# googlegenomics/spark-examples

Hardware: NVIDIA H100
Metric: genotype-cells/sec (N x V) into Gram (higher is better)
Workload: dtype int8

## Files before the change

include/vpca.h:

```cpp
#ifndef VPCA_H_
#define VPCA_H_

#include <stddef.h>
#include <stdint.h>

#ifdef __cplusplus
extern "C" {
#endif

#define VPCA_VERSION_MAJOR 0
#define VPCA_VERSION_MINOR 2

typedef enum vpca_status {
    VPCA_OK = 0,
    VPCA_ERR_BAD_ARG = -1,
    VPCA_ERR_INDEX_OUT_OF_RANGE = -2,
    VPCA_ERR_CUDA = -3,
    VPCA_ERR_NCCL = -4,
    VPCA_ERR_OVERFLOW = -5,
    VPCA_ERR_STATE = -6,
    VPCA_ERR_NOMEM = -7,
    VPCA_ERR_UNSUPPORTED = -8
} vpca_status;

// ... 152 lines not shown
    int32_t eig_method;
    int32_t eig_iterations;
} vpca_stats;
int vpca_get_stats(vpca_ctx* ctx, vpca_stats* out);
int vpca_debug_gram_profile(vpca_ctx* ctx, int64_t* out, int32_t max_ctas);
int vpca_debug_lanczos_profile(vpca_ctx* ctx, int64_t* out, int32_t max_steps);

#define VPCA_JOIN 0
#define VPCA_MERGE 1
int vpca_hash_keys(vpca_ctx* ctx, const uint8_t* payload, const int64_t* key_offsets, int64_t nkeys, uint64_t* out);
int vpca_join_rows(vpca_ctx* ctx, int32_t mode, int32_t variant_set_count, int64_t n_left, const uint8_t* key_payload,
                   const int64_t* key_offsets, const int64_t* offsets, const int32_t* sample_idx, int64_t nrows,
                   int64_t* out_rows, int64_t* out_nnz);
int vpca_join_fetch(vpca_ctx* ctx, int64_t* out_offsets, int32_t* out_idx);
int vpca_join_size(vpca_ctx* ctx, int64_t* out_rows, int64_t* out_nnz);
int vpca_accumulate_joined(vpca_ctx* ctx, int64_t partition_id);

int vpca_debug_rebalance(const int32_t* tiles, int32_t num_tiles, int32_t workers, int32_t kb_window, int32_t col_limit,
                         double* cum, int32_t* out, int32_t max_pieces);
int vpca_debug_tiles(int32_t n_samples, int32_t cta_group, int32_t exact, int32_t* out, int32_t max_tiles);
int vpca_debug_band_tiles(int32_t n_samples, int32_t cta_group, int32_t row0, int32_t rows, int32_t* out, int32_t max_tiles);
int vpca_debug_max_clusters(int32_t device, int32_t cluster_size);
int vpca_debug_plan(const int32_t* tiles, int32_t num_tiles, int32_t workers, int32_t kb_window, int32_t* out, int32_t max_pieces);

#ifdef __cplusplus
}
#endif
#endif
```

spark_examples_b200/csrc/gram_sm90.cu:

```cuda
#include <cuda.h>
#include <cuda_runtime.h>

#include <cstring>

#include <algorithm>
#include <map>
#include <mutex>
#include <tuple>
#include <type_traits>
#include <cstdio>
#include <cstdlib>
#include <string>
#include <vector>

#include "ptx_sm90.cuh"
#include "vpca_internal.h"

namespace vpca {

namespace {

constexpr int kThreads = 384;
constexpr int kKBytes = 128;
constexpr int kBoxRows = 128;
// ... 29 lines not shown
struct GramArgs {
    int32_t* S;
    int32_t* peer[kMaxPeers];
    int num_peers;
    int peer_mode;
    int own_end[kMaxPeers];
    const TileDesc* tiles;
    int* err;
    int n;
    int num_tiles;
    int num_full;
    int total_weight;
    int kb_total;
    int kb_window;
    int num_workers;
    int resident;
    int kc_per_kb;
    int kb_per_panel;
    int sync_lead;
    int active_workers;
    int* win_done;
    long long* prof;
    const double* cum;
    int col_limit;
    int acc_stride;
    int row_limit;
    int red64;
};

struct Seg {
    int tile, kb0, kb1, col, slot, first, flush, use, win, last_in_win;
    int rowA0, rowA1, rowB, n_eff, flags;
};

struct SegPlan {
    int n;
    int tile[kMaxSegs], lo[kMaxSegs], hi[kMaxSegs], col[kMaxSegs];
    int cols;
    int overflow;
};

__host__ __device__ inline void plan_segments(const TileDesc* tiles, int num_tiles, int first_tile, long long u_begin,
                                              long long u_end, int len, SegPlan& p) {
    p.n = 0;
    p.cols = 0;
    p.overflow = 0;
// ... 67 lines not shown
            int h = 0;
            if (feasible_end(tiles, num_tiles, mid, need[j + 1], len, col_limit, h) >= need[j + 1]) hi = mid;
            else lo = mid + 1;
        }
        need[j] = hi;
    }
    long long ub = 0;
    int hint = 0;
    for (int i = 0; i < workers; ++i) {
        long long ue = (i + 1 == workers) ? uw : (long long)((double)uw * cand[i + 1]);
        if (ue < ub) ue = ub;
        if (i + 1 < workers && ue < need[i + 1]) ue = need[i + 1];
        const long long fe = feasible_end(tiles, num_tiles, ub, ue, len, col_limit, hint);
        if (fe < ue) {
            if (i + 1 == workers || fe < need[i + 1]) return false;
            ue = fe;
        }
        if (i + 1 < workers) cand[i + 1] = ((double)ue + 0.5) / (double)uw;
        ub = ue;
    }
    return true;
}

struct Sched {
    SegPlan plan;
    long long u_begin, u_end, u;
    int kbw, nwin, kb_total, resident, win, seg_i, nflush, acc_stride;
    int worker, workers, num_tiles, wave, full_waves, tail_first;
    const TileDesc* tiles;

    __device__ void init(const GramArgs& a, int w) {
        kbw = a.kb_window;
        kb_total = a.kb_total;
        resident = a.resident;
        acc_stride = a.acc_stride;
        worker = w;
        workers = a.num_workers;
        num_tiles = a.num_tiles;
        tiles = a.tiles;
        nwin = (kb_total + kbw - 1) / kbw;
        win = 0;
        seg_i = 0;
        nflush = 0;
        wave = 0;
        if (resident) {
            const long long uw = (long long)a.total_weight * kbw;
            u_begin = (long long)((double)uw * a.cum[worker]);
            u_end = (worker + 1 == a.num_workers) ? uw : (long long)((double)uw * a.cum[worker + 1]);
            plan_segments(tiles, num_tiles, 0, u_begin, u_end, kbw, plan);
            if (plan.overflow || plan.cols > a.col_limit) {
                if (a.err != nullptr && threadIdx.x == 0) {
                    a.err[0] = 9;
                    a.err[1] = (int)blockIdx.x;
                    a.err[2] = plan.cols;
                    a.err[3] = plan.n;
                    __threadfence_system();
                }
                __trap();
            }
        } else {
            full_waves = a.num_full / workers;
            tail_first = full_waves * workers;
            const long long tail_units =
                tail_first < num_tiles ? (long long)(a.total_weight - tiles[tail_first].wstart) * kb_total : 0;
            u_begin = tail_units * worker / workers;
            u_end = tail_units * (worker + 1) / workers;
            plan.n = 0;
        }
        u = u_begin;
    }
    __device__ void fill(Seg& s, int t) const {
        const int4 lo = __ldg(reinterpret_cast<const int4*>(tiles + t));
        const int4 hi = __ldg(reinterpret_cast<const int4*>(tiles + t) + 1);
        s.tile = t;
        s.rowA0 = lo.x;
        s.rowA1 = lo.y;
        s.rowB = lo.z;
        s.n_eff = lo.w;
        s.flags = hi.y;
    }
    __device__ bool next(Seg& s) {
        if (!resident) {
            s.win = 0;
            s.last_in_win = 0;
            s.first = 1;
            s.flush = 1;
            s.slot = nflush & 1;
            s.col = s.slot * acc_stride;
            s.use = nflush >> 1;
            if (wave < full_waves) {
                fill(s, wave * workers + worker);
                s.kb0 = 0;
                s.kb1 = kb_total;
                ++wave;
                ++nflush;
                return true;
            }
            while (true) {
                if (seg_i < plan.n) {
                    fill(s, plan.tile[seg_i]);
                    s.kb0 = plan.lo[seg_i];
                    s.kb1 = plan.hi[seg_i];
                    ++seg_i;
                    ++nflush;
                    return true;
                }
                if (u >= u_end) return false;
                plan_segments(tiles, num_tiles, tail_first, u, u_end, kb_total, plan);
                seg_i = 0;
                if (plan.n == 0) return false;
                const int lt = plan.tile[plan.n - 1];
                const long long base = (long long)(tiles[lt].wstart - tiles[tail_first].wstart) * kb_total;
                const long long endu = base + (long long)plan.hi[plan.n - 1] * (tiles[lt].n_eff >> 4);
                u = plan.overflow ? endu : u_end;
            }
        }
        if (plan.n == 0) return false;
        if (seg_i == plan.n) {
            ++win;
            seg_i = 0;
        }
        if (win >= nwin) return false;
        const int i = seg_i++;
        fill(s, plan.tile[i]);
        const int base = win * kbw;
        const int cnt = min(kbw, kb_total - base);
        s.kb0 = base + min(plan.lo[i], cnt);
        s.kb1 = base + min(plan.hi[i], cnt);
        s.win = win;
        s.last_in_win = (seg_i == plan.n);
        s.col = plan.col[i];
        s.slot = i;
        s.first = (win == 0);
        s.flush = (win == nwin - 1);
        s.use = 0;
        return true;
    }
};

__device__ __forceinline__ void mbar_wait(uint32_t bar, uint32_t parity, int* err, int code) {
    if (ptx::mbar_try_wait(bar, parity)) return;
    const long long t0 = clock64();
    while (!ptx::mbar_try_wait(bar, parity)) {
        if (clock64() - t0 > kWatchdogCycles) {
            if (err != nullptr) {
                err[0] = code;
                err[1] = (int)blockIdx.x;
                err[2] = (int)bar;
                err[3] = (int)parity;
                __threadfence_system();
            }
// ... 345 lines not shown
        double acc = 0.0;
        cand[0] = 0.0;
        for (int i = 0; i < workers; ++i) {
            acc += sh[i] / sum;
            cand[i + 1] = (i + 1 == workers) ? 1.0 : acc;
        }
    }
    __syncthreads();
    if (active) {
        const long long uw = (long long)total_weight * kbw;
        const long long ub = (long long)((double)uw * cand[w]);
        const long long ue = (w + 1 == workers) ? uw : (long long)((double)uw * cand[w + 1]);
        int hint = 0;
        if (feasible_end(tiles, num_tiles, ub, ue, kbw, col_limit, hint) < ue) atomicExch(&need_repair, 1);
    }
    __syncthreads();
    if (need_repair && w == 0 && !repair_split(tiles, num_tiles, workers, (long long)total_weight * kbw, kbw, col_limit, cand, need)) reject = 1;
    __syncthreads();
    if (reject) return;
    if (w <= workers) cum[w] = cand[w];
    if (w == 0) *gen += 1;
}

__global__ void symmetrize_kernel(int32_t* __restrict__ S, int n) {
    __shared__ int32_t tile[32][33];
    const int bx = blockIdx.x, by = blockIdx.y;
    if (bx < by) return;
    const int tx = threadIdx.x, ty = threadIdx.y;
    for (int r = ty; r < 32; r += 8) {
        const int row = bx * 32 + r, col = by * 32 + tx;
        tile[r][tx] = (row < n && col < n) ? S[(size_t)row * n + col] : 0;
    }
    __syncthreads();
    for (int r = ty; r < 32; r += 8) {
        const int row = by * 32 + r, col = bx * 32 + tx;
        if (row < n && col < n && row < col) S[(size_t)row * n + col] = tile[tx][r];
    }
}

__global__ void add_i32_kernel(int32_t* __restrict__ dst, const int32_t* __restrict__ src, int64_t count) {
    int64_t i = (int64_t)blockIdx.x * blockDim.x + threadIdx.x;
    const int64_t stride = (int64_t)gridDim.x * blockDim.x;
    for (; i < count; i += stride) dst[i] += src[i];
}

struct PeerPtrs {
// ... 152 lines not shown
    if (cudaOccupancyMaxActiveClusters(&clusters, gram_kernel<2, KIND>, &cfg) != cudaSuccess) {
        cudaGetLastError();
        return -1;
    }
    return clusters;
}

}

namespace {
struct SplitKey {
    int dev, n, tiles, kbw, workers, elem;
    bool operator<(const SplitKey& o) const {
        return std::tie(dev, n, tiles, kbw, workers, elem) < std::tie(o.dev, o.n, o.tiles, o.kbw, o.workers, o.elem);
    }
};
std::mutex g_split_mu;
std::map<SplitKey, std::vector<double>> g_splits;
}

static void remember_split(GramPlan& plan) {
    if (plan.d_cum == nullptr || plan.cum_workers <= 0 || !plan.adaptive) return;
    if (plan.own_hi > plan.own_lo && plan.num_peers <= 1) return;
    std::vector<double> cum((size_t)plan.cum_workers + 1);
    if (cudaMemcpy(cum.data(), plan.d_cum, cum.size() * sizeof(double), cudaMemcpyDeviceToHost) != cudaSuccess) {
        cudaGetLastError();
        return;
    }
    std::lock_guard<std::mutex> lk(g_split_mu);
    g_splits[SplitKey{plan.cum_dev, plan.cum_for_n, plan.cum_tiles, plan.cum_kbw, plan.cum_workers, plan.cum_elem}] = std::move(cum);
}

void gram_plan_free(GramPlan& plan) {
    remember_split(plan);
    if (plan.d_tiles) cudaFree(plan.d_tiles);
    plan.h_tiles.clear();
    if (plan.d_err) cudaFreeHost(plan.d_err);
    if (plan.d_win_done) cudaFree(plan.d_win_done);
    if (plan.d_prof) cudaFree(plan.d_prof);
    if (plan.d_cum) cudaFree(plan.d_cum);
    plan.d_cum = nullptr;
    plan.d_win_done = nullptr;
    plan.d_prof = nullptr;
    plan.d_tiles = nullptr;
    plan.d_err = nullptr;
    plan.tiles_for_n = -1;
}
// ... 99 lines not shown
    int num_full = 0;
    make_tiles(n, plan.cta_group, exact, BN, row_lo, row_hi, plan.self_b, tiles, &num_full);
    if (plan.d_tiles) cudaFree(plan.d_tiles);
    plan.d_tiles = nullptr;
    cudaError_t e = cudaMalloc(&plan.d_tiles, tiles.size() * sizeof(TileDesc));
    if (e != cudaSuccess) return e;
    e = cudaMemcpyAsync(plan.d_tiles, tiles.data(), tiles.size() * sizeof(TileDesc), cudaMemcpyHostToDevice, stream);
    if (e != cudaSuccess) return e;
    e = cudaStreamSynchronize(stream);
    plan.h_tiles.assign(reinterpret_cast<const int32_t*>(tiles.data()),
                        reinterpret_cast<const int32_t*>(tiles.data() + tiles.size()));
    plan.num_tiles = (int)tiles.size();
    plan.num_full = num_full;
    plan.total_weight = tiles.empty() ? 0 : tiles.back().wstart + (tiles.back().n_eff >> 4);
    plan.tiles_for_n = n;
    plan.tiles_for_cg = plan.cta_group;
    plan.tiles_for_bn = exact ? -1 : BN;
    plan.tiles_row_lo = row_lo;
    plan.tiles_row_hi = row_hi;
    plan.tiles_col_limit = kAccCols;
    return e;
}

static bool initial_split(const GramPlan& plan, int workers, int kbw, std::vector<double>& cum) {
    if (plan.total_weight <= 0) return false;
    const TileDesc* tiles = reinterpret_cast<const TileDesc*>(plan.h_tiles.data());
    const long long uw = (long long)plan.total_weight * kbw;
    cum.resize((size_t)workers + 1);
    for (int w = 0; w <= workers; ++w) cum[w] = (double)w / (double)workers;
    std::vector<long long> need((size_t)workers + 1);
    if (!repair_split(tiles, plan.num_tiles, workers, uw, kbw, plan.tiles_col_limit, cum.data(), need.data())) return false;
    for (int w = 0; w < workers; ++w) {
        const long long ub = (long long)((double)uw * cum[w]);
        const long long ue = (w + 1 == workers) ? uw : (long long)((double)uw * cum[w + 1]);
        SegPlan p;
        plan_segments(tiles, plan.num_tiles, 0, ub, ue, kbw, p);
        if (p.overflow || p.cols > plan.tiles_col_limit) return false;
    }
    return true;
}

int gram_debug_tiles(int n, int cta_group, int exact, int32_t* out, int max_tiles) {
    std::vector<TileDesc> tiles;
    int num_full = 0;
    make_tiles(n, cta_group == 1 ? 1 : 2, exact != 0, kUmmaN, 0, n, true, tiles, &num_full);
    const int cnt = std::min<int>((int)tiles.size(), max_tiles);
// ... 17 lines not shown
    for (int w = 0; w <= workers; ++w) cum[w] = (double)w / (double)workers;
    return gram_debug_repair(tiles8, num_tiles, workers, kbw, col_limit, cum.data(), out, max_pieces);
}

int gram_debug_repair(const int32_t* tiles8, int num_tiles, int workers, int kbw, int col_limit, double* cum, int32_t* out,
                      int max_pieces) {
    const TileDesc* tiles = reinterpret_cast<const TileDesc*>(tiles8);
    if (num_tiles <= 0) return 0;
    const long long total = tiles[num_tiles - 1].wstart + (tiles[num_tiles - 1].n_eff >> 4);
    const long long uw = total * kbw;
    std::vector<long long> need((size_t)workers + 1);
    if (!repair_split(tiles, num_tiles, workers, uw, kbw, col_limit, cum, need.data())) return -1000;
    int cnt = 0;
    for (int w = 0; w < workers; ++w) {
        const long long ub = (long long)((double)uw * cum[w]);
        const long long ue = (w + 1 == workers) ? uw : (long long)((double)uw * cum[w + 1]);
        SegPlan p;
        plan_segments(tiles, num_tiles, 0, ub, ue, kbw, p);
        if (p.overflow || p.cols > col_limit) return -1 - w;
        for (int i = 0; i < p.n; ++i, ++cnt)
            if (cnt < max_pieces) {
                int32_t* o = out + (size_t)cnt * 6;
                o[0] = w; o[1] = p.tile[i]; o[2] = p.lo[i]; o[3] = p.hi[i]; o[4] = p.col[i]; o[5] = p.cols;
            }
    }
    return cnt;
}

cudaError_t gram_accumulate(GramPlan& plan, const void* d_x, int elem_bits, int n, int64_t nv, int64_t ld, int64_t panel,
                            int32_t* d_S, cudaStream_t stream, std::string* err) {
    if (nv <= 0) return cudaSuccess;
    EncodeTiledFn encode = get_encode_fn();
    if (encode == nullptr) {
        if (err) *err = "cuTensorMapEncodeTiled entry point not available";
        return cudaErrorNotSupported;
    }
    if (plan.num_sms == 0) {
        int dev = 0;
        cudaGetDevice(&dev);
        cudaDeviceGetAttribute(&plan.num_sms, cudaDevAttrMultiProcessorCount, dev);
        const char* cg = getenv("VPCA_CTA_GROUP");
        if (cg != nullptr) plan.cta_group = (atoi(cg) == 1) ? 1 : 2;
        const char* kw = getenv("VPCA_KB_WINDOW");
        if (kw != nullptr) plan.kb_window = atoi(kw);
        const char* sl = getenv("VPCA_SYNC_LEAD");
        if (sl != nullptr) plan.sync_lead = atoi(sl);
// ... 82 lines not shown
        return cudaErrorInvalidValue;
    }

    GramArgs args{};
    args.S = banded ? d_S - (ptrdiff_t)plan.own_lo * n : d_S;
    args.num_peers = (plan.num_peers > 1 && d_S == plan.peer_base[plan.peer_rank]) ? plan.num_peers : 0;
    for (int d = 0; d < kMaxPeers; ++d) args.peer[d] = d < plan.num_peers ? plan.peer_S[d] : nullptr;
    args.peer_mode = plan.peer_mode;
    for (int d = 0; d < kMaxPeers; ++d) args.own_end[d] = plan.own_end[d];
    args.tiles = static_cast<const TileDesc*>(plan.d_tiles);
    cudaHostGetDevicePointer(reinterpret_cast<void**>(&args.err), plan.d_err, 0);
    args.n = n;
    args.num_tiles = plan.num_tiles;
    args.num_full = plan.num_full;
    args.total_weight = plan.total_weight;
    args.kb_total = (int)((nv + elems_per_kb - 1) / elems_per_kb);
    args.kb_per_panel = panel > 0 ? (int)(panel / elems_per_kb) : args.kb_total;
    args.num_workers = workers;
    args.kc_per_kb = kc_per_kb;
    args.acc_stride = 0;
    args.col_limit = plan.tiles_col_limit;
    args.row_limit = row_hi;
    args.red64 = plan.red64 ? 1 : 0;
    {
        int kbw = plan.kb_window;
        if (kbw <= 0 && panel > 0) kbw = args.kb_per_panel;
        if (kbw <= 0) {
            const long long target = 16ll << 20;
            kbw = (int)std::max<long long>(8, std::min<long long>(4096, target / ((long long)n * kKBytes)));
        }
        kbw = std::min(kbw, args.kb_total);
        std::vector<double> cum0;
        args.resident = (plan.num_tiles <= 4 * workers && initial_split(plan, workers, kbw, cum0)) ? 1 : 0;
        int dev = 0;
        cudaGetDevice(&dev);
        args.kb_window = args.resident ? kbw : args.kb_total;
        if (args.resident && (plan.d_cum == nullptr || plan.cum_workers != workers || plan.cum_tiles != plan.num_tiles ||
                              plan.cum_kbw != kbw || plan.cum_for_n != n || plan.cum_elem != elem_bits)) {
            remember_split(plan);
            if (plan.adaptive && !banded) {
                std::lock_guard<std::mutex> lk(g_split_mu);
                auto it = g_splits.find(SplitKey{dev, n, plan.num_tiles, kbw, workers, elem_bits});
                if (it != g_splits.end()) {
                    std::vector<double> learned = it->second;
                    const TileDesc* tiles = reinterpret_cast<const TileDesc*>(plan.h_tiles.data());
                    std::vector<long long> need((size_t)workers + 1);
                    if (repair_split(tiles, plan.num_tiles, workers, (long long)plan.total_weight * kbw, kbw, plan.tiles_col_limit,
                                     learned.data(), need.data()))
                        cum0 = learned;
                }
            }
            if (plan.d_cum) cudaFree(plan.d_cum);
            plan.d_cum = nullptr;
            cudaError_t e = cudaMalloc(&plan.d_cum, (size_t)(workers + 2) * sizeof(double) + sizeof(int));
            if (e != cudaSuccess) return e;
            cum0.push_back(0.0);
            cum0.push_back(0.0);
            e = cudaMemcpyAsync(plan.d_cum, cum0.data(), (size_t)(workers + 2) * sizeof(double) + sizeof(int),
                                cudaMemcpyHostToDevice, stream);
            if (e != cudaSuccess) return e;
            plan.cum_workers = workers;
            plan.cum_tiles = plan.num_tiles;
            plan.cum_kbw = kbw;
            plan.cum_for_n = n;
            plan.cum_dev = dev;
            plan.cum_elem = elem_bits;
        }
    }
    plan.last_resident = args.resident;
    const int nwin = (args.kb_total + args.kb_window - 1) / args.kb_window;
    const long long uw = (long long)args.total_weight * args.kb_window;
    args.active_workers = (int)std::min<long long>(workers, uw);
    args.sync_lead = (args.resident && nwin <= GramPlan::kMaxWindows) ? plan.sync_lead : 0;
    args.win_done = plan.d_win_done;
    const bool adapt = plan.adaptive && args.resident && workers <= 1024 && args.active_workers == workers;
    args.prof = (plan.profile || adapt) ? plan.d_prof : nullptr;
    args.cum = plan.d_cum;
    if (args.sync_lead > 0) {
        cudaError_t e = cudaMemsetAsync(plan.d_win_done, 0, (size_t)nwin * sizeof(int), stream);
        if (e != cudaSuccess) return e;
    }

    const int grid = workers * cgp;
    cudaError_t le;
    if (cgp == 2)
        le = kind == 0 ? launch<2, 0>(tmap, args, grid, stream)
                       : (kind == 1 ? launch<2, 1>(tmap, args, grid, stream) : launch<2, 2>(tmap, args, grid, stream));
    else
        le = kind == 0 ? launch<1, 0>(tmap, args, grid, stream)
                       : (kind == 1 ? launch<1, 1>(tmap, args, grid, stream) : launch<1, 2>(tmap, args, grid, stream));
    if (le != cudaSuccess) return le;
    if (adapt) {
        rebalance_kernel<<<1, 1024, 0, stream>>>(plan.d_prof, plan.d_cum, workers, cgp, plan.gain, 1.35, 300000,
                                                 reinterpret_cast<int*>(plan.d_cum + workers + 2), static_cast<const TileDesc*>(plan.d_tiles), plan.num_tiles,
                                                 plan.total_weight, args.kb_window, plan.tiles_col_limit);
        le = cudaGetLastError();
    }
    return le;
}

cudaError_t gram_preload_kernels(cudaStream_t stream) {
    cudaFuncAttributes fa;
    cudaError_t e = cudaSuccess;
#define VPCA_LOAD(k) if (e == cudaSuccess) e = cudaFuncGetAttributes(&fa, k)
    VPCA_LOAD((gram_kernel<1, 0>)); VPCA_LOAD((gram_kernel<1, 1>)); VPCA_LOAD((gram_kernel<1, 2>));
    VPCA_LOAD((gram_kernel<2, 0>)); VPCA_LOAD((gram_kernel<2, 1>)); VPCA_LOAD((gram_kernel<2, 2>));
    VPCA_LOAD(rebalance_kernel); VPCA_LOAD(symmetrize_kernel); VPCA_LOAD(add_i32_kernel); VPCA_LOAD(add_i32_peers_kernel);
    VPCA_LOAD(add_i32_owner_kernel); VPCA_LOAD(gather_rows_kernel); VPCA_LOAD(push_rows_kernel); VPCA_LOAD(peer_barrier_kernel);
#undef VPCA_LOAD
    if (e != cudaSuccess) return e;
    PeerPtrs pp{};
    OwnEnds own{};
    peer_barrier_kernel<<<1, 32, 0, stream>>>(pp, 0, 0, 0);
    push_rows_kernel<<<1, 32, 0, stream>>>(pp, nullptr, own, 0, 0, 0);
    gather_rows_kernel<<<1, 32, 0, stream>>>(pp, nullptr, own, 0, 0, 0);
    add_i32_owner_kernel<<<1, 32, 0, stream>>>(pp, own, 0, nullptr, 0);
    add_i32_peers_kernel<<<1, 32, 0, stream>>>(pp, 0, nullptr, 0);
    add_i32_kernel<<<1, 32, 0, stream>>>(nullptr, nullptr, 0);
    symmetrize_kernel<<<dim3(1, 1), dim3(32, 8), 0, stream>>>(nullptr, 0);
    return cudaGetLastError();
}

int gram_debug_max_clusters(int cluster_size) { return max_clusters<0>(cluster_size); }

cudaError_t gram_symmetrize(int32_t* d_S, int n, cudaStream_t stream) {
    const int nb = (n + 31) / 32;
    symmetrize_kernel<<<dim3(nb, nb), dim3(32, 8), 0, stream>>>(d_S, n);
    return cudaGetLastError();
}

// ... 54 lines not shown
```

spark_examples_b200/csrc/vpca.cu:

```cuda
#include <cuda_runtime.h>

#include <algorithm>
#include <atomic>
#include <cmath>
#include <condition_variable>
#include <cstdarg>
#include <cstdio>
#include <cstring>
#include <functional>
#include <mutex>
#include <string>
#include <thread>
#include <vector>

#include "vpca_internal.h"

using namespace vpca;

namespace {
thread_local std::string tls_error;
thread_local const vpca_ctx* tls_error_ctx = nullptr;
thread_local std::string tls_error_copy;
}

// ... 2558 lines not shown
}

int vpca_debug_max_clusters(int32_t device, int32_t cluster_size) {
    if (cluster_size < 1 || cluster_size > 16) return fail(nullptr, VPCA_ERR_BAD_ARG, "cluster_size must be in [1, 16]");
    if (cudaSetDevice(device) != cudaSuccess) return fail(nullptr, VPCA_ERR_CUDA, "cudaSetDevice(%d) failed", device);
    const int c = gram_debug_max_clusters(cluster_size);
    if (c < 0) return fail(nullptr, VPCA_ERR_CUDA, "cudaOccupancyMaxActiveClusters failed for cluster size %d", cluster_size);
    return c;
}

int vpca_debug_tiles(int32_t n_samples, int32_t cta_group, int32_t exact, int32_t* out, int32_t max_tiles) {
    if (n_samples < 2 || max_tiles < 0) return fail(nullptr, VPCA_ERR_BAD_ARG, "vpca_debug_tiles: bad argument");
    return gram_debug_tiles(n_samples, cta_group, exact, out, max_tiles);
}

int vpca_debug_plan(const int32_t* tiles, int32_t num_tiles, int32_t workers, int32_t kb_window, int32_t* out, int32_t max_pieces) {
    if (tiles == nullptr || num_tiles < 1 || workers < 1 || kb_window < 1 || (out == nullptr && max_pieces > 0))
        return fail(nullptr, VPCA_ERR_BAD_ARG, "vpca_debug_plan: bad argument");
    const int rc = gram_debug_plan(tiles, num_tiles, workers, kb_window, out, max_pieces);
    if (rc < 0) return fail(nullptr, VPCA_ERR_STATE, "vpca_debug_plan: the accumulators of a worker do not fit its budget (large-N schedule)");
    return rc;
}

int vpca_debug_rebalance(const int32_t* tiles, int32_t num_tiles, int32_t workers, int32_t kb_window, int32_t col_limit,
                         double* cum, int32_t* out, int32_t max_pieces) {
    if (tiles == nullptr || num_tiles < 1 || workers < 1 || kb_window < 1 || cum == nullptr || col_limit < 32 ||
        (out == nullptr && max_pieces > 0))
        return fail(nullptr, VPCA_ERR_BAD_ARG, "vpca_debug_rebalance: bad argument");
    const int rc = gram_debug_repair(tiles, num_tiles, workers, kb_window, col_limit, cum, out, max_pieces);
    if (rc < 0) return fail(nullptr, VPCA_ERR_STATE, "vpca_debug_rebalance: no feasible repair of this split");
    return rc;
}

int vpca_host_alloc(size_t bytes, void** out) {
    if (out == nullptr || bytes == 0) return fail(nullptr, VPCA_ERR_BAD_ARG, "vpca_host_alloc: bad argument");
    cudaError_t e = cudaHostAlloc(out, bytes, cudaHostAllocPortable);
    if (e != cudaSuccess) {
        *out = nullptr;
        return fail(nullptr, VPCA_ERR_NOMEM, "cudaHostAlloc(%zu): %s", bytes, cudaGetErrorString(e));
    }
    return VPCA_OK;
}

int vpca_host_free(void* p) {
    if (p == nullptr) return VPCA_OK;
    cudaError_t e = cudaFreeHost(p);
// ... 6 lines not shown
```

spark_examples_b200/csrc/vpca_internal.h:

```cpp
#pragma once
#include <cstdint>
#include <cuda_runtime.h>
#include <string>
#include <vector>

#include "../../include/vpca.h"

namespace vpca {

struct GramPlan {
    int cta_group = 2;
    int kb_window = 0;
    int num_sms = 0;
    int max_pairs[3] = {};
    void* d_tiles = nullptr;
    std::vector<int32_t> h_tiles;
    int num_tiles = 0;
    int num_full = 0;
    int total_weight = 0;
    int tiles_col_limit = 256;
    bool exact_cover = false;
    int tiles_for_n = -1;
    int tiles_for_cg = 0;
    int tiles_for_bn = 0;
// ... 18 lines not shown
    bool peers_ipc = false;
    int peer_mode = 0;
    int own_end[16] = {};
    bool profile = false;
    long long* d_prof = nullptr;
};
int gram_read_profile(GramPlan& plan, long long* out, int max_ctas);

cudaError_t gram_accumulate(GramPlan& plan, const void* d_x, int elem_bits, int n, int64_t nv, int64_t ld, int64_t panel,
                            int32_t* d_S, cudaStream_t stream, std::string* err);
cudaError_t gram_symmetrize(int32_t* d_S, int n, cudaStream_t stream);
cudaError_t gram_add(int32_t* d_dst, const int32_t* d_src, int64_t count, cudaStream_t stream);
cudaError_t gram_add_peers(GramPlan& plan, const int32_t* d_src, int64_t count, cudaStream_t stream);
cudaError_t gram_add_owners(GramPlan& plan, const int32_t* d_src, int n, cudaStream_t stream);
cudaError_t gram_gather_rows(GramPlan& plan, int32_t* d_S, int n, cudaStream_t stream);
cudaError_t gram_peer_barrier(GramPlan& plan, cudaStream_t stream);
cudaError_t gram_preload_kernels(cudaStream_t stream);
cudaError_t encode_preload_kernels();
void gram_plan_free(GramPlan& plan);
int gram_debug_max_clusters(int cluster_size);
int gram_debug_band_tiles(int n, int cta_group, int row_lo, int row_hi, int32_t* out, int max_tiles);
int gram_debug_tiles(int n, int cta_group, int exact, int32_t* out, int max_tiles);
int gram_debug_plan(const int32_t* tiles8, int num_tiles, int workers, int kbw, int32_t* out, int max_pieces);
int gram_debug_repair(const int32_t* tiles8, int num_tiles, int workers, int kbw, int col_limit, double* cum, int32_t* out,
                      int max_pieces);

cudaError_t encode_calls(const int64_t* d_off, int64_t base, const void* d_idx, int idx_bytes, int64_t nv, int n,
                         int elem_bits, int max_mult, void* d_x, int64_t ld, int64_t panel, int* d_flags,
                         cudaStream_t stream);

cudaError_t encode_bits(const uint8_t* d_bits, int64_t stride, int64_t nv, int n, int elem_bits, void* d_x, int64_t ld,
                        int64_t panel, int code, cudaStream_t stream);

cudaError_t encode_bed_planes(const uint8_t* d_rows, int64_t stride, int64_t nv, int n, void* d_x, int64_t panel,
                              cudaStream_t stream);

cudaError_t encode_ld_planes(const uint8_t* d_rows, int64_t pitch, int64_t width, int nv, int c, int64_t s0, int64_t len,
                             int n, void* d_x, int64_t panel, cudaStream_t stream);

constexpr int kLdMaxWindow = VPCA_LD_MAX_WINDOW;
constexpr int kLdMaxChunk = 2 * kLdMaxWindow;
struct LdChunk {
    const int32_t* G;
    const int64_t* wlo;
    int64_t s0;
    int c, nc, own_lo, T;
// ... 165 lines not shown
```

spark_examples_b200/native.py:

```python
from __future__ import annotations

import ctypes
import os
from pathlib import Path
from typing import Optional, Tuple

import numpy as np

VPCA_OK = 0
VPCA_ERR_BAD_ARG = -1
VPCA_ERR_INDEX_OUT_OF_RANGE = -2
VPCA_ERR_CUDA = -3
VPCA_ERR_NCCL = -4
VPCA_ERR_OVERFLOW = -5
VPCA_ERR_STATE = -6
VPCA_ERR_NOMEM = -7
VPCA_ERR_UNSUPPORTED = -8
JOIN, MERGE = 0, 1

DTYPE_I8 = 0
DTYPE_BF16 = 1
DTYPE_E2M1 = 2

_STATUS_NAMES = {
    -1: "BAD_ARG", -2: "INDEX_OUT_OF_RANGE", -3: "CUDA", -4: "NCCL", -5: "OVERFLOW", -6: "STATE",
    -7: "NOMEM", -8: "UNSUPPORTED",
}

EXPORTED_SYMBOLS = (
    "vpca_version", "vpca_create", "vpca_destroy", "vpca_last_error", "vpca_reset", "vpca_encode_calls",
    "vpca_accumulate_calls", "vpca_commit", "vpca_abort", "vpca_accumulate_dense", "vpca_gram_device_ptr",
    "vpca_finalize_gram", "vpca_get_gram", "vpca_set_gram", "vpca_compute_pca", "vpca_get_centered",
    "vpca_get_tridiagonal", "vpca_synth_dense_device", "vpca_get_stats", "vpca_debug_gram_profile",
    "vpca_gram_export_ipc", "vpca_gram_set_peers", "vpca_peer_barrier", "vpca_accumulate_panels",
    "vpca_synth_panels_device", "vpca_accumulate_calls_u16", "vpca_get_partial_gram", "vpca_load_partial_gram",
    "vpca_accumulate_bits", "vpca_gram_set_peer_mode", "vpca_gram_gather", "vpca_accumulate_bed",
    "vpca_synchronize", "vpca_host_alloc", "vpca_host_free", "vpca_gram_set_peers_local", "vpca_owner_row_bands",
    "vpca_get_gram_band", "vpca_variant_count", "vpca_debug_rebalance",
    "vpca_debug_lanczos_profile", "vpca_debug_max_clusters", "vpca_debug_band_tiles", "vpca_hash_keys", "vpca_join_rows", "vpca_join_fetch", "vpca_join_size", "vpca_accumulate_joined",
    "vpca_pool_create", "vpca_pool_destroy", "vpca_pool_size", "vpca_pool_ctx", "vpca_pool_last_error", "vpca_pool_reset",
    "vpca_pool_accumulate_calls", "vpca_pool_accumulate_calls_u16", "vpca_pool_accumulate_bits", "vpca_pool_accumulate_bed",
    "vpca_pool_commit", "vpca_pool_abort", "vpca_pool_reduce_and_finalize", "vpca_pool_get_gram", "vpca_pool_compute_pca",
    "vpca_pool_get_stats", "vpca_debug_tiles", "vpca_debug_plan",
    "vpca_loadings_calls", "vpca_loadings_bed", "vpca_loadings_panels", "vpca_project_begin", "vpca_project_calls",
    "vpca_project_bed", "vpca_project_panels", "vpca_project_get", "vpca_compute_pca_bands",
    "vpca_kinship_bed", "vpca_kinship_pairs", "vpca_compute_pca_subset", "vpca_ld_prune_bed",
    "vpca_ld_prune_bed_masked", "vpca_variant_qc_bed", "vpca_hwe_exact", "vpca_sample_missing_bed",
    "vpca_subset_bed_samples",
)

KINSHIP_MAX_SAMPLES = 21845
LD_MAX_WINDOW = 4096


class VpcaError(RuntimeError):

    def __init__(self, code: int, message: str):
        super().__init__(f"vpca {_STATUS_NAMES.get(code, code)}: {message}")
        self.code = code


class IndexOutOfRange(VpcaError, IndexError):
    """Sample index outside [0, N): the reference throws at VariantsPca.scala:59 / :188."""


class VpcaConfig(ctypes.Structure):
# ... 126 lines not shown
    L.vpca_pool_accumulate_calls.argtypes = [vp, i64, vp, vp, i64]
    L.vpca_pool_accumulate_calls_u16.restype = ctypes.c_int
    L.vpca_pool_accumulate_calls_u16.argtypes = [vp, i64, vp, vp, i64]
    L.vpca_pool_accumulate_bits.restype = ctypes.c_int
    L.vpca_pool_accumulate_bits.argtypes = [vp, i64, vp, i64, i64]
    L.vpca_pool_accumulate_bed.restype = ctypes.c_int
    L.vpca_pool_accumulate_bed.argtypes = [vp, i64, vp, i64, i64, i32]
    L.vpca_pool_commit.restype = ctypes.c_int
    L.vpca_pool_commit.argtypes = [vp, i64]
    L.vpca_pool_abort.restype = ctypes.c_int
    L.vpca_pool_abort.argtypes = [vp, i64]
    L.vpca_pool_reduce_and_finalize.restype = ctypes.c_int
    L.vpca_pool_reduce_and_finalize.argtypes = [vp]
    L.vpca_pool_get_gram.restype = ctypes.c_int
    L.vpca_pool_get_gram.argtypes = [vp, vp]
    L.vpca_pool_compute_pca.restype = ctypes.c_int
    L.vpca_pool_compute_pca.argtypes = [vp, i32, vp, vp, ctypes.POINTER(i32)]
    L.vpca_pool_get_stats.restype = ctypes.c_int
    L.vpca_pool_get_stats.argtypes = [vp, ctypes.POINTER(VpcaStats)]
    L.vpca_debug_tiles.restype = ctypes.c_int
    L.vpca_debug_tiles.argtypes = [i32, i32, i32, vp, i32]
    L.vpca_debug_plan.restype = ctypes.c_int
    L.vpca_debug_plan.argtypes = [vp, i32, i32, i32, vp, i32]
    L.vpca_debug_lanczos_profile.restype = ctypes.c_int
    L.vpca_debug_lanczos_profile.argtypes = [vp, vp, i32]
    L.vpca_debug_rebalance.restype = ctypes.c_int
    L.vpca_debug_rebalance.argtypes = [vp, i32, i32, i32, i32, vp, vp, i32]
    L.vpca_set_gram.restype = ctypes.c_int
    L.vpca_set_gram.argtypes = [vp, vp]
    L.vpca_compute_pca.restype = ctypes.c_int
    L.vpca_compute_pca.argtypes = [vp, i32, vp, vp, ctypes.POINTER(i32)]
    L.vpca_compute_pca_bands.restype = ctypes.c_int
    L.vpca_compute_pca_bands.argtypes = [ctypes.POINTER(vp), i32, i32, vp, vp, ctypes.POINTER(i32)]
    L.vpca_get_centered.restype = ctypes.c_int
    L.vpca_get_centered.argtypes = [vp, vp]
    L.vpca_get_tridiagonal.restype = ctypes.c_int
    L.vpca_get_tridiagonal.argtypes = [vp, vp, vp]
    L.vpca_synth_dense_device.restype = ctypes.c_int
    L.vpca_synth_dense_device.argtypes = [vp, ctypes.c_uint64, i64, i64, ctypes.c_int, vp, i64]
    L.vpca_get_stats.restype = ctypes.c_int
    L.vpca_get_stats.argtypes = [vp, ctypes.POINTER(VpcaStats)]
    L.vpca_accumulate_panels.restype = ctypes.c_int
    L.vpca_accumulate_panels.argtypes = [vp, vp, i64, i64]
    L.vpca_synth_panels_device.restype = ctypes.c_int
    L.vpca_synth_panels_device.argtypes = [vp, ctypes.c_uint64, i64, i64, ctypes.c_int, vp, i64]
    L.vpca_gram_export_ipc.restype = ctypes.c_int
# ... 506 lines not shown


def debugTiles(n_samples: int, cta_group: int = 2, exact: bool = True) -> np.ndarray:
    L = load_library()
    cnt = L.vpca_debug_tiles(int(n_samples), int(cta_group), 1 if exact else 0, None, 0)
    if cnt < 0:
        raise VpcaError(cnt, L.vpca_last_error(None).decode("utf-8", "replace"))
    out = np.zeros((cnt, 8), dtype=np.int32)
    L.vpca_debug_tiles(int(n_samples), int(cta_group), 1 if exact else 0, _host_ptr(out), cnt)
    return out


def debugPlan(tiles: np.ndarray, workers: int, kb_window: int) -> np.ndarray:
    L = load_library()
    t = np.ascontiguousarray(tiles, dtype=np.int32)
    cap = 8 * int(workers) + 8
    out = np.zeros((cap, 6), dtype=np.int32)
    cnt = L.vpca_debug_plan(_host_ptr(t), len(t), int(workers), int(kb_window), _host_ptr(out), cap)
    if cnt < 0:
        raise VpcaError(VPCA_ERR_STATE, L.vpca_last_error(None).decode("utf-8", "replace"))
    return out[:cnt]


def debugBandTiles(n_samples: int, cta_group: int, row0: int, rows: int) -> np.ndarray:
    L = load_library()
    L.vpca_debug_band_tiles.restype = ctypes.c_int
    L.vpca_debug_band_tiles.argtypes = [ctypes.c_int32] * 4 + [ctypes.c_void_p, ctypes.c_int32]
    cnt = L.vpca_debug_band_tiles(int(n_samples), int(cta_group), int(row0), int(rows), None, 0)
    if cnt < 0:
        raise VpcaError(cnt, L.vpca_last_error(None).decode("utf-8", "replace"))
    out = np.zeros((cnt, 8), dtype=np.int32)
    L.vpca_debug_band_tiles(int(n_samples), int(cta_group), int(row0), int(rows), _host_ptr(out), cnt)
    return out


def maxClusters(device: int, cluster_size: int) -> int:
    L = load_library()
    L.vpca_debug_max_clusters.restype = ctypes.c_int
    L.vpca_debug_max_clusters.argtypes = [ctypes.c_int32, ctypes.c_int32]
    c = L.vpca_debug_max_clusters(int(device), int(cluster_size))
    if c < 0:
        raise VpcaError(c, L.vpca_last_error(None).decode("utf-8", "replace"))
    return c


def debugRebalance(tiles: np.ndarray, workers: int, kb_window: int, cum: np.ndarray, col_limit: int = 512):
# ... 149 lines not shown
```

Before: 534.8 billion.

## Add front/tail split schedule for tile counts between half and all workers

When the number of Gram tiles is between half and the full worker count, each tile gets a dedicated front worker for the first fraction of the K blocks. The remaining K range of all tiles is spread evenly across the idle tail workers and accumulated with flush. A new rebalance kernel adjusts the split fraction from measured per-side times, and the learned fraction is remembered across calls. This targets idle SMs when tiles are fewer than workers, at the cost of extra partial-sum flushes and schedule complexity.

```diff
diff --git a/include/vpca.h b/include/vpca.h
--- a/include/vpca.h
+++ b/include/vpca.h
@@ -198,6 +198,8 @@
 int vpca_debug_band_tiles(int32_t n_samples, int32_t cta_group, int32_t row0, int32_t rows, int32_t* out, int32_t max_tiles);
 int vpca_debug_max_clusters(int32_t device, int32_t cluster_size);
 int vpca_debug_plan(const int32_t* tiles, int32_t num_tiles, int32_t workers, int32_t kb_window, int32_t* out, int32_t max_pieces);
+int vpca_debug_schedule(int32_t n_samples, int32_t cta_group, int32_t exact, int32_t workers, int32_t kb_window,
+                        int32_t kb_total, double front_frac, int32_t* out, int32_t max_pieces, int32_t* info);
 
 #ifdef __cplusplus
 }
diff --git a/spark_examples_b200/csrc/gram_sm90.cu b/spark_examples_b200/csrc/gram_sm90.cu
--- a/spark_examples_b200/csrc/gram_sm90.cu
+++ b/spark_examples_b200/csrc/gram_sm90.cu
@@ -75,6 +75,8 @@
     int* win_done;
     long long* prof;
     const double* cum;
+    int front_tiles;
+    const double* front_frac;
     int col_limit;
     int acc_stride;
     int row_limit;
@@ -188,33 +190,67 @@
     return true;
 }
 
+__host__ __device__ inline bool front_tail_applies(int num_tiles, int workers) {
+    return 2 * num_tiles > workers && num_tiles < workers;
+}
+
+__host__ __device__ inline int front_split(double frac, int kb_total) {
+    const double f = frac < 0.0 ? 0.0 : (frac > 1.0 ? 1.0 : frac);
+    const int s = (int)(f * (double)kb_total);
+    return s < kb_total ? s : kb_total;
+}
+
 struct Sched {
     SegPlan plan;
     long long u_begin, u_end, u;
-    int kbw, nwin, kb_total, resident, win, seg_i, nflush, acc_stride;
+    int kbw, nwin, kb_total, kb_end, resident, win, seg_i, nflush, acc_stride;
     int worker, workers, num_tiles, wave, full_waves, tail_first;
+    int tail, kb_split;
     const TileDesc* tiles;
 
-    __device__ void init(const GramArgs& a, int w) {
+    __host__ __device__ bool init(const GramArgs& a, int w) {
         kbw = a.kb_window;
         kb_total = a.kb_total;
+        kb_end = kb_total;
         resident = a.resident;
         acc_stride = a.acc_stride;
         worker = w;
         workers = a.num_workers;
         num_tiles = a.num_tiles;
         tiles = a.tiles;
-        nwin = (kb_total + kbw - 1) / kbw;
         win = 0;
         seg_i = 0;
         nflush = 0;
         wave = 0;
-        if (resident) {
+        tail = 0;
+        kb_split = kb_total;
+        u_begin = u_end = 0;
+        if (a.front_tiles > 0) {
+            kb_split = front_split(*a.front_frac, kb_total);
+            if (worker < a.front_tiles) {
+                kb_end = kb_split;
+                plan.n = 1;
+                plan.tile[0] = worker;
+                plan.lo[0] = 0;
+                plan.hi[0] = kbw;
+                plan.col[0] = 0;
+                plan.cols = tiles[worker].acc_cols;
+                plan.overflow = 0;
+            } else {
+                tail = 1;
+                const long long units = (long long)a.front_tiles * (kb_total - kb_split);
+                const int tw = workers - a.front_tiles, j = worker - a.front_tiles;
+                u_begin = units * j / tw;
+                u_end = units * (j + 1) / tw;
+                plan.n = 0;
+            }
+        } else if (resident) {
             const long long uw = (long long)a.total_weight * kbw;
             u_begin = (long long)((double)uw * a.cum[worker]);
             u_end = (worker + 1 == a.num_workers) ? uw : (long long)((double)uw * a.cum[worker + 1]);
             plan_segments(tiles, num_tiles, 0, u_begin, u_end, kbw, plan);
             if (plan.overflow || plan.cols > a.col_limit) {
+#ifdef __CUDA_ARCH__
                 if (a.err != nullptr && threadIdx.x == 0) {
                     a.err[0] = 9;
                     a.err[1] = (int)blockIdx.x;
@@ -223,6 +259,9 @@
                     __threadfence_system();
                 }
                 __trap();
+#else
+                return false;
+#endif
             }
         } else {
             full_waves = a.num_full / workers;
@@ -233,11 +272,18 @@
             u_end = tail_units * (worker + 1) / workers;
             plan.n = 0;
         }
+        nwin = (kb_end + kbw - 1) / kbw;
         u = u_begin;
-    }
-    __device__ void fill(Seg& s, int t) const {
+        return true;
+    }
+    __host__ __device__ void fill(Seg& s, int t) const {
+#ifdef __CUDA_ARCH__
         const int4 lo = __ldg(reinterpret_cast<const int4*>(tiles + t));
         const int4 hi = __ldg(reinterpret_cast<const int4*>(tiles + t) + 1);
+#else
+        const int4 lo = reinterpret_cast<const int4*>(tiles + t)[0];
+        const int4 hi = reinterpret_cast<const int4*>(tiles + t)[1];
+#endif
         s.tile = t;
         s.rowA0 = lo.x;
         s.rowA1 = lo.y;
@@ -245,7 +291,25 @@
         s.n_eff = lo.w;
         s.flags = hi.y;
     }
-    __device__ bool next(Seg& s) {
+    __host__ __device__ bool next(Seg& s) {
+        if (tail) {
+            if (u >= u_end) return false;
+            const int span = kb_total - kb_split;
+            const int t = (int)(u / span);
+            const long long e = u_end < (long long)(t + 1) * span ? u_end : (long long)(t + 1) * span;
+            fill(s, t);
+            s.kb0 = kb_split + (int)(u - (long long)t * span);
+            s.kb1 = kb_split + (int)(e - (long long)t * span);
+            s.win = -1;
+            s.last_in_win = 0;
+            s.first = 1;
+            s.flush = 1;
+            s.col = 0;
+            s.slot = 0;
+            s.use = 0;
+            u = e;
+            return true;
+        }
         if (!resident) {
             s.win = 0;
             s.last_in_win = 0;
@@ -290,9 +354,9 @@
         const int i = seg_i++;
         fill(s, plan.tile[i]);
         const int base = win * kbw;
-        const int cnt = min(kbw, kb_total - base);
-        s.kb0 = base + min(plan.lo[i], cnt);
-        s.kb1 = base + min(plan.hi[i], cnt);
+        const int cnt = kbw < kb_end - base ? kbw : kb_end - base;
+        s.kb0 = base + (plan.lo[i] < cnt ? plan.lo[i] : cnt);
+        s.kb1 = base + (plan.hi[i] < cnt ? plan.hi[i] : cnt);
         s.win = win;
         s.last_in_win = (seg_i == plan.n);
         s.col = plan.col[i];
@@ -684,6 +748,42 @@
     if (w == 0) *gen += 1;
 }
 
+__global__ void rebalance_front_kernel(const long long* __restrict__ prof, double* __restrict__ frac, int front, int workers,
+                                       int cta_group, int kb_total, double gain, double lo, double hi, long long min_ns,
+                                       int* __restrict__ gen) {
+    __shared__ long long tmax[2][32];
+    const int w = threadIdx.x;
+    long long t = 0;
+    if (w < workers) t = prof[(size_t)w * cta_group * 4 + 2] - prof[(size_t)w * cta_group * 4 + 0];
+    const int side = w < front ? 0 : 1;
+    long long m0 = side == 0 ? t : 0, m1 = side == 1 ? t : 0;
+    for (int o = 16; o > 0; o >>= 1) {
+        m0 = max(m0, __shfl_xor_sync(0xffffffffu, m0, o));
+        m1 = max(m1, __shfl_xor_sync(0xffffffffu, m1, o));
+    }
+    if ((w & 31) == 0) {
+        tmax[0][w >> 5] = m0;
+        tmax[1][w >> 5] = m1;
+    }
+    __syncthreads();
+    if (w != 0) return;
+    long long tf = 0, tt = 0;
+    for (int i = 0; i < (int)(blockDim.x >> 5); ++i) {
+        tf = max(tf, tmax[0][i]);
+        tt = max(tt, tmax[1][i]);
+    }
+    const double f = *frac;
+    const int s = front_split(f, kb_total);
+    if (s <= 0 || s >= kb_total) return;
+    if (tf < min_ns || tt < min_ns) return;
+    if (llabs(tf - tt) < (max(tf, tt) >> 8)) return;
+    const double a = (double)tf / (double)s, b = (double)tt / (double)(kb_total - s);
+    const double target = b / (a + b);
+    const double nf = fmin(fmax((1.0 - gain) * f + gain * target, lo), hi);
+    *frac = nf;
+    *gen += 1;
+}
+
 __global__ void symmetrize_kernel(int32_t* __restrict__ S, int n) {
     __shared__ int32_t tile[32][33];
     const int bx = blockIdx.x, by = blockIdx.y;
@@ -882,7 +982,7 @@
 static void remember_split(GramPlan& plan) {
     if (plan.d_cum == nullptr || plan.cum_workers <= 0 || !plan.adaptive) return;
     if (plan.own_hi > plan.own_lo && plan.num_peers <= 1) return;
-    std::vector<double> cum((size_t)plan.cum_workers + 1);
+    std::vector<double> cum((size_t)plan.cum_workers + 2);
     if (cudaMemcpy(cum.data(), plan.d_cum, cum.size() * sizeof(double), cudaMemcpyDeviceToHost) != cudaSuccess) {
         cudaGetLastError();
         return;
@@ -1028,6 +1128,22 @@
     return e;
 }
 
+struct FrontRange {
+    bool on = false;
+    double init = 0.0, lo = 0.0, hi = 0.0;
+};
+
+static FrontRange front_range(int num_tiles, int workers, bool banded) {
+    FrontRange r;
+    r.on = !banded && front_tail_applies(num_tiles, workers);
+    if (r.on) {
+        r.init = (double)num_tiles / (double)workers;
+        r.lo = 0.5 * r.init;
+        r.hi = r.init + 0.5 * (1.0 - r.init);
+    }
+    return r;
+}
+
 static bool initial_split(const GramPlan& plan, int workers, int kbw, std::vector<double>& cum) {
     if (plan.total_weight <= 0) return false;
     const TileDesc* tiles = reinterpret_cast<const TileDesc*>(plan.h_tiles.data());
@@ -1091,6 +1207,53 @@
             if (cnt < max_pieces) {
                 int32_t* o = out + (size_t)cnt * 6;
                 o[0] = w; o[1] = p.tile[i]; o[2] = p.lo[i]; o[3] = p.hi[i]; o[4] = p.col[i]; o[5] = p.cols;
+            }
+    }
+    return cnt;
+}
+
+int gram_debug_schedule(int n, int cta_group, int exact, int workers, int kbw, int kb_total, double frac, int32_t* out,
+                        int max_pieces, int32_t* info) {
+    GramPlan plan;
+    plan.cta_group = cta_group == 1 ? 1 : 2;
+    std::vector<TileDesc> tiles;
+    int num_full = 0;
+    make_tiles(n, plan.cta_group, exact != 0, kUmmaN, 0, n, true, tiles, &num_full);
+    plan.h_tiles.assign(reinterpret_cast<const int32_t*>(tiles.data()), reinterpret_cast<const int32_t*>(tiles.data() + tiles.size()));
+    plan.num_tiles = (int)tiles.size();
+    plan.num_full = num_full;
+    plan.total_weight = tiles.back().wstart + (tiles.back().n_eff >> 4);
+    kbw = std::min(kbw, kb_total);
+    std::vector<double> cum;
+    const FrontRange front = front_range(plan.num_tiles, workers, false);
+    GramArgs a{};
+    a.tiles = tiles.data();
+    a.n = n;
+    a.num_tiles = plan.num_tiles;
+    a.num_full = num_full;
+    a.total_weight = plan.total_weight;
+    a.kb_total = kb_total;
+    a.num_workers = workers;
+    a.col_limit = plan.tiles_col_limit;
+    a.resident = front.on || (plan.num_tiles <= 4 * workers && initial_split(plan, workers, kbw, cum)) ? 1 : 0;
+    a.kb_window = a.resident ? kbw : kb_total;
+    a.cum = cum.data();
+    const double f = frac >= 0.0 ? frac : front.init;
+    if (front.on) {
+        a.front_tiles = plan.num_tiles;
+        a.front_frac = &f;
+    }
+    info[0] = front.on ? 2 : a.resident;
+    info[1] = front.on ? front_split(f, kb_total) : kb_total;
+    int cnt = 0;
+    for (int w = 0; w < workers; ++w) {
+        Sched sc;
+        if (!sc.init(a, w)) return -1 - w;
+        Seg s;
+        for (; sc.next(s); ++cnt)
+            if (cnt < max_pieces) {
+                int32_t* o = out + (size_t)cnt * 6;
+                o[0] = w; o[1] = s.tile; o[2] = s.kb0; o[3] = s.kb1; o[4] = s.first; o[5] = s.flush;
             }
     }
     return cnt;
@@ -1219,6 +1382,7 @@
     args.col_limit = plan.tiles_col_limit;
     args.row_limit = row_hi;
     args.red64 = plan.red64 ? 1 : 0;
+    FrontRange front;
     {
         int kbw = plan.kb_window;
         if (kbw <= 0 && panel > 0) kbw = args.kb_per_panel;
@@ -1228,7 +1392,14 @@
         }
         kbw = std::min(kbw, args.kb_total);
         std::vector<double> cum0;
-        args.resident = (plan.num_tiles <= 4 * workers && initial_split(plan, workers, kbw, cum0)) ? 1 : 0;
+        front = front_range(plan.num_tiles, workers, banded);
+        if (front.on) {
+            args.resident = 1;
+            cum0.assign((size_t)workers + 1, 0.0);
+        } else {
+            args.resident = (plan.num_tiles <= 4 * workers && initial_split(plan, workers, kbw, cum0)) ? 1 : 0;
+        }
+        double frac0 = front.init;
         int dev = 0;
         cudaGetDevice(&dev);
         args.kb_window = args.resident ? kbw : args.kb_total;
@@ -1240,18 +1411,24 @@
                 auto it = g_splits.find(SplitKey{dev, n, plan.num_tiles, kbw, workers, elem_bits});
                 if (it != g_splits.end()) {
                     std::vector<double> learned = it->second;
-                    const TileDesc* tiles = reinterpret_cast<const TileDesc*>(plan.h_tiles.data());
-                    std::vector<long long> need((size_t)workers + 1);
-                    if (repair_split(tiles, plan.num_tiles, workers, (long long)plan.total_weight * kbw, kbw, plan.tiles_col_limit,
-                                     learned.data(), need.data()))
-                        cum0 = learned;
+                    if (front.on) {
+                        const double f = learned.size() > (size_t)workers + 1 ? learned[(size_t)workers + 1] : -1.0;
+                        if (f >= front.lo && f <= front.hi) frac0 = f;
+                    } else {
+                        const TileDesc* tiles = reinterpret_cast<const TileDesc*>(plan.h_tiles.data());
+                        std::vector<long long> need((size_t)workers + 1);
+                        learned.resize((size_t)workers + 1);
+                        if (repair_split(tiles, plan.num_tiles, workers, (long long)plan.total_weight * kbw, kbw,
+                                         plan.tiles_col_limit, learned.data(), need.data()))
+                            cum0 = learned;
+                    }
                 }
             }
             if (plan.d_cum) cudaFree(plan.d_cum);
             plan.d_cum = nullptr;
             cudaError_t e = cudaMalloc(&plan.d_cum, (size_t)(workers + 2) * sizeof(double) + sizeof(int));
             if (e != cudaSuccess) return e;
-            cum0.push_back(0.0);
+            cum0.push_back(frac0);
             cum0.push_back(0.0);
             e = cudaMemcpyAsync(plan.d_cum, cum0.data(), (size_t)(workers + 2) * sizeof(double) + sizeof(int),
                                 cudaMemcpyHostToDevice, stream);
@@ -1268,9 +1445,14 @@
     const int nwin = (args.kb_total + args.kb_window - 1) / args.kb_window;
     const long long uw = (long long)args.total_weight * args.kb_window;
     args.active_workers = (int)std::min<long long>(workers, uw);
+    if (front.on) {
+        args.front_tiles = plan.num_tiles;
+        args.front_frac = plan.d_cum + workers + 1;
+        args.active_workers = plan.num_tiles;
+    }
     args.sync_lead = (args.resident && nwin <= GramPlan::kMaxWindows) ? plan.sync_lead : 0;
     args.win_done = plan.d_win_done;
-    const bool adapt = plan.adaptive && args.resident && workers <= 1024 && args.active_workers == workers;
+    const bool adapt = plan.adaptive && args.resident && workers <= 1024 && (front.on || args.active_workers == workers);
     args.prof = (plan.profile || adapt) ? plan.d_prof : nullptr;
     args.cum = plan.d_cum;
     if (args.sync_lead > 0) {
@@ -1287,7 +1469,12 @@
         le = kind == 0 ? launch<1, 0>(tmap, args, grid, stream)
                        : (kind == 1 ? launch<1, 1>(tmap, args, grid, stream) : launch<1, 2>(tmap, args, grid, stream));
     if (le != cudaSuccess) return le;
-    if (adapt) {
+    if (adapt && front.on) {
+        rebalance_front_kernel<<<1, (workers + 31) / 32 * 32, 0, stream>>>(
+            plan.d_prof, plan.d_cum + workers + 1, plan.num_tiles, workers, cgp, args.kb_total, plan.gain, front.lo, front.hi,
+            300000, reinterpret_cast<int*>(plan.d_cum + workers + 2));
+        le = cudaGetLastError();
+    } else if (adapt) {
         rebalance_kernel<<<1, 1024, 0, stream>>>(plan.d_prof, plan.d_cum, workers, cgp, plan.gain, 1.35, 300000,
                                                  reinterpret_cast<int*>(plan.d_cum + workers + 2), static_cast<const TileDesc*>(plan.d_tiles), plan.num_tiles,
                                                  plan.total_weight, args.kb_window, plan.tiles_col_limit);
@@ -1302,7 +1489,7 @@
 #define VPCA_LOAD(k) if (e == cudaSuccess) e = cudaFuncGetAttributes(&fa, k)
     VPCA_LOAD((gram_kernel<1, 0>)); VPCA_LOAD((gram_kernel<1, 1>)); VPCA_LOAD((gram_kernel<1, 2>));
     VPCA_LOAD((gram_kernel<2, 0>)); VPCA_LOAD((gram_kernel<2, 1>)); VPCA_LOAD((gram_kernel<2, 2>));
-    VPCA_LOAD(rebalance_kernel); VPCA_LOAD(symmetrize_kernel); VPCA_LOAD(add_i32_kernel); VPCA_LOAD(add_i32_peers_kernel);
+    VPCA_LOAD(rebalance_kernel); VPCA_LOAD(rebalance_front_kernel); VPCA_LOAD(symmetrize_kernel); VPCA_LOAD(add_i32_kernel); VPCA_LOAD(add_i32_peers_kernel);
     VPCA_LOAD(add_i32_owner_kernel); VPCA_LOAD(gather_rows_kernel); VPCA_LOAD(push_rows_kernel); VPCA_LOAD(peer_barrier_kernel);
 #undef VPCA_LOAD
     if (e != cudaSuccess) return e;
diff --git a/spark_examples_b200/csrc/vpca.cu b/spark_examples_b200/csrc/vpca.cu
--- a/spark_examples_b200/csrc/vpca.cu
+++ b/spark_examples_b200/csrc/vpca.cu
@@ -2604,6 +2604,16 @@
     return rc;
 }
 
+int vpca_debug_schedule(int32_t n_samples, int32_t cta_group, int32_t exact, int32_t workers, int32_t kb_window,
+                        int32_t kb_total, double front_frac, int32_t* out, int32_t max_pieces, int32_t* info) {
+    if (n_samples < 2 || workers < 1 || workers > 1024 || kb_window < 1 || kb_total < 1 || !(front_frac <= 1.0) ||
+        info == nullptr || max_pieces < 0 || (out == nullptr && max_pieces > 0))
+        return fail(nullptr, VPCA_ERR_BAD_ARG, "vpca_debug_schedule: bad argument");
+    const int rc = gram_debug_schedule(n_samples, cta_group, exact, workers, kb_window, kb_total, front_frac, out, max_pieces, info);
+    if (rc < 0) return fail(nullptr, VPCA_ERR_STATE, "vpca_debug_schedule: the accumulators of a worker do not fit its budget");
+    return rc;
+}
+
 int vpca_debug_rebalance(const int32_t* tiles, int32_t num_tiles, int32_t workers, int32_t kb_window, int32_t col_limit,
                          double* cum, int32_t* out, int32_t max_pieces) {
     if (tiles == nullptr || num_tiles < 1 || workers < 1 || kb_window < 1 || cum == nullptr || col_limit < 32 ||
diff --git a/spark_examples_b200/csrc/vpca_internal.h b/spark_examples_b200/csrc/vpca_internal.h
--- a/spark_examples_b200/csrc/vpca_internal.h
+++ b/spark_examples_b200/csrc/vpca_internal.h
@@ -64,6 +64,8 @@
 int gram_debug_band_tiles(int n, int cta_group, int row_lo, int row_hi, int32_t* out, int max_tiles);
 int gram_debug_tiles(int n, int cta_group, int exact, int32_t* out, int max_tiles);
 int gram_debug_plan(const int32_t* tiles8, int num_tiles, int workers, int kbw, int32_t* out, int max_pieces);
+int gram_debug_schedule(int n, int cta_group, int exact, int workers, int kbw, int kb_total, double frac, int32_t* out,
+                        int max_pieces, int32_t* info);
 int gram_debug_repair(const int32_t* tiles8, int num_tiles, int workers, int kbw, int col_limit, double* cum, int32_t* out,
                       int max_pieces);
 
diff --git a/spark_examples_b200/native.py b/spark_examples_b200/native.py
--- a/spark_examples_b200/native.py
+++ b/spark_examples_b200/native.py
@@ -41,7 +41,7 @@
     "vpca_pool_create", "vpca_pool_destroy", "vpca_pool_size", "vpca_pool_ctx", "vpca_pool_last_error", "vpca_pool_reset",
     "vpca_pool_accumulate_calls", "vpca_pool_accumulate_calls_u16", "vpca_pool_accumulate_bits", "vpca_pool_accumulate_bed",
     "vpca_pool_commit", "vpca_pool_abort", "vpca_pool_reduce_and_finalize", "vpca_pool_get_gram", "vpca_pool_compute_pca",
-    "vpca_pool_get_stats", "vpca_debug_tiles", "vpca_debug_plan",
+    "vpca_pool_get_stats", "vpca_debug_tiles", "vpca_debug_plan", "vpca_debug_schedule",
     "vpca_loadings_calls", "vpca_loadings_bed", "vpca_loadings_panels", "vpca_project_begin", "vpca_project_calls",
     "vpca_project_bed", "vpca_project_panels", "vpca_project_get", "vpca_compute_pca_bands",
     "vpca_kinship_bed", "vpca_kinship_pairs", "vpca_compute_pca_subset", "vpca_ld_prune_bed",
@@ -214,6 +214,8 @@
     L.vpca_debug_tiles.argtypes = [i32, i32, i32, vp, i32]
     L.vpca_debug_plan.restype = ctypes.c_int
     L.vpca_debug_plan.argtypes = [vp, i32, i32, i32, vp, i32]
+    L.vpca_debug_schedule.restype = ctypes.c_int
+    L.vpca_debug_schedule.argtypes = [i32, i32, i32, i32, i32, i32, ctypes.c_double, vp, i32, vp]
     L.vpca_debug_lanczos_profile.restype = ctypes.c_int
     L.vpca_debug_lanczos_profile.argtypes = [vp, vp, i32]
     L.vpca_debug_rebalance.restype = ctypes.c_int
@@ -766,6 +768,20 @@
     return out[:cnt]
 
 
+def debugSchedule(n_samples: int, cta_group: int, exact: bool, workers: int, kb_window: int, kb_total: int,
+                  front_frac: float = -1.0):
+    L = load_library()
+    info = np.zeros(2, dtype=np.int32)
+    args = (int(n_samples), int(cta_group), 1 if exact else 0, int(workers), int(kb_window), int(kb_total),
+            float(front_frac))
+    cnt = L.vpca_debug_schedule(*args, None, 0, _host_ptr(info))
+    if cnt < 0:
+        raise VpcaError(cnt, L.vpca_last_error(None).decode("utf-8", "replace"))
+    out = np.zeros((cnt, 6), dtype=np.int32)
+    L.vpca_debug_schedule(*args, _host_ptr(out), cnt, _host_ptr(info))
+    return out, int(info[0]), int(info[1])
+
+
 def debugBandTiles(n_samples: int, cta_group: int, row0: int, rows: int) -> np.ndarray:
     L = load_library()
     L.vpca_debug_band_tiles.restype = ctypes.c_int
```

Result: faster. 626.8 billion, median of 6 (+17.2%).
